# Corleno/Nonstationary_Multivariate_Gaussian_Process

Measured on AMD Instinct MI355X. Metric: log-posterior evals/sec (N=2048, D=3 nonseparable GP), higher is better.
Workload: dtype f64

## Files before the change

nonstationary_multivariate_gaussian_process_amd/csrc/nmgp_chol.hip:

```cpp
#include "nmgp_internal.h"
#include <cstring>

namespace nmgpk {

static inline int cdiv_c(long long a, long long b) { return (int)((a + b - 1) / b); }

typedef double v4d __attribute__((ext_vector_type(4)));

#define SY_BM 128
#define SY_BK 16
#define SY_LD (SY_BM + 16)
#define SY_SB 8

__device__ __forceinline__ int clamp_row_pair(int r, int rows) {
    int rc = r < rows - 1 ? r : rows - 2;
    return rc < 0 ? 0 : rc;
}

__device__ __forceinline__ double fast_recip(double p) {
    double x = __builtin_amdgcn_rcp(p);
    double e = fma(-p, x, 1.0);
    x = fma(x, e, x);
    e = fma(-p, x, 1.0);
    x = fma(x, e, x);
// ... 1542 lines not shown
#pragma unroll
        for (int kk = 0; kk < 4; ++kk) x0 = __builtin_amdgcn_mfma_f64_16x16x4f64(ai[kk], T[pp][kk], x0, 0, 0, 0);
        T[pp] = x0;
#pragma unroll
        for (int kk = 0; kk < 4; ++kk)
#pragma unroll
            for (int q = pp + 1; q < 4; ++q) {
                const double a = reinterpret_cast<const double*>(&ops[(q == 1 ? 0 : (q == 2 ? 1 : 3)) + pp][lane])[kk];
                T[q] = __builtin_amdgcn_mfma_f64_16x16x4f64(a, T[pp][kk], T[q], 0, 0, 0);
            }
    }
    if (v0) {
#pragma unroll
        for (int q = 0; q < 4; ++q)
#pragma unroll
            for (int r = 0; r < 4; ++r) A[(size_t)(16 * q + 4 * r + l4) * lda + row] = T[q][r];
    }
}

static void trsm_64(hipStream_t s, const double* L, int ldl, int nb, double* A, int lda, int rows, int batch,
                    long long bstride, bool precise) {
    if (rows <= 0) return;
    if (precise) {
        NMGP_LAUNCH(k_trsm_64, dim3(cdiv_c(rows, 64), batch), dim3(256), 0, s, L, ldl, nb, A, lda, rows, bstride);
    } else if (nb == 64) {
        NMGP_LAUNCH(k_trsm_64h<5>, dim3(cdiv_c(rows, 64), batch), dim3(256), 0, s, L, ldl, A, lda, rows, bstride);
    } else {
        const long long wgs = (long long)cdiv_c(rows, 128) * batch;
        const int reps = wgs >= 4096 ? 4 : (wgs >= 2048 ? 2 : 1);
        NMGP_LAUNCH(k_trsm_64m, dim3(cdiv_c(rows, 128 * reps), batch), dim3(256), 0, s, L, ldl, nb, A, lda, rows, bstride, reps);
    }
}

#define PS_XLD 66
#define PS_XPS_OFF 6656
#define PS_XS_OFF (PS_XPS_OFF + 64 * PS_XLD)
#define PS_SMEM_DOUBLES (PS_XS_OFF + 64 * PS_XLD)

template <int MODE, int OCC = 2>
__global__ __launch_bounds__(512, OCC) void k_panel_step(double* __restrict__ Ab, int lda, int ck, int has_prev_a,
                                                        int has_next_a,
                                                        int m_act, int pend, long long bstride, int* __restrict__ info,
                                                        int istride, int T, int u_mrows, int u_ncols, int u_kflags,
                                                        int u_tiles, int nbatch, int pre_a, int un_fresh, int u_tri,
                                                        long long* __restrict__ stamps) {
    const int has_prev = MODE == 0 ? has_prev_a : (MODE == 2 ? 1 : 0);
    const int has_next = MODE == 0 ? has_next_a : (MODE == 1 ? 1 : 0);
    const int pre = MODE == 0 ? pre_a : 0;
    constexpr int kOpsT = MODE == 1 ? 0 : 4096;
    constexpr int kXps = PS_XPS_OFF;
    constexpr int kXs = MODE == 1 ? 2560 : PS_XS_OFF;
    constexpr int kSmem = MODE == 1 ? 2560 + 64 * PS_XLD
                                    : (MODE == 2 ? 6656 : (PS_SMEM_DOUBLES > 4 * SY_BK * SY_LD ? PS_SMEM_DOUBLES : 4 * SY_BK * SY_LD));
    static_assert(MODE != 1 || sizeof(Potf2Lds) <= kSmem * sizeof(double), "the factorisation's LDS aliases the step's");
#define PS_STAMP(i)                                                              \
    do {                                                                         \
        if (stamps && blockIdx.x == 0 && threadIdx.x == 0) stamps[i] = (long long)wall_clock64(); \
    } while (0)
    PS_STAMP(0);
    __shared__ __attribute__((aligned(32))) double smem[kSmem];
    const int tid = threadIdx.x, lane = tid & 63, w = tid >> 6;
    const int l15 = lane & 15, l4 = lane >> 4;
    const int bx = (int)blockIdx.x / nbatch, by = (int)blockIdx.x - bx * nbatch;
    if (bx >= T) {
        if constexpr (MODE == 0) {
            const int t = bx - T + by * u_tiles;
            const double* Ap = Ab + (size_t)(ck - 64) * lda + (ck + 128);
            double* Cp = Ab + (size_t)(ck + 128) * lda + (ck + 128);
            syrk_tile_body<4, SY_BK>(Ap, lda, Cp, lda, u_mrows, u_ncols, 64, bstride, bstride, u_kflags, -u_tiles, nbatch, t, 0,
                                     0, smem, smem + 2 * SY_BK * SY_LD, u_tri, 0);
        }
        return;
    }
    double* A = Ab + (size_t)by * bstride;
    v4d* opsC = reinterpret_cast<v4d*>(smem);
    v4d* opsT = reinterpret_cast<v4d*>(smem + kOpsT);
    double* Xps = smem + (MODE == 0 ? kXps : 0);
    double* Xs = smem + (MODE == 2 ? 0 : kXs);
    const bool wg0 = bx == 0;
    const bool isC = wg0 && w < 4;
    const bool wg1 = pre && bx == 1;
    const bool isP = wg1 && w < 4;
    const int row = wg0 ? ck + 64 + 16 * w + l15 : ck + 128 + 128 * (bx - 1) + 16 * w + l15;
    const bool rv = row < m_act && !(wg0 && w >= 4);
    const int rowc = row < m_act ? row : (m_act - 1);
    const bool un_used = has_next && (has_prev || wg0);
    double oc[8], ot[5];
    v4d Xp[4], Tk[4], Un[4];
    const double* Lp = A + (size_t)(ck - 64) * lda;
    if (has_prev) {
#pragma unroll
        for (int j = 0; j < 8; ++j) {
            const int e = tid + 512 * j, q = e >> 10, sx = (e >> 6) & 15, l = e & 63;
            oc[j] = -Lp[(size_t)(4 * sx + (l >> 4)) * lda + ck + 16 * q + (l & 15)];
        }
    }
    {
        const double* L = A + (size_t)ck * lda + ck;
#pragma unroll
        for (int j = 0; j < 5; ++j) {
            const int idx = tid + 512 * j;
            const int blk = idx >> 8, kk = (idx >> 6) & 3, l = idx & 63;
            const int rr = l & 15, kc = 4 * kk + (l >> 4);
            double v;
            if (blk < 6) {
                const int q = blk == 0 ? 1 : (blk < 3 ? 2 : 3);
                const int pp = blk == 0 ? 0 : (blk < 3 ? blk - 1 : blk - 3);
                v = -L[(size_t)(16 * pp + kc) * lda + 16 * q + rr];
            } else {
                const int q = blk - 6;
                if (kc < rr) v = L[(size_t)(16 * q + rr) * lda + 16 * q + kc];
                else if (kc == rr) v = 1.0 / L[(size_t)(16 * q + rr) * lda + 16 * q + rr];
                else v = 0.0;
            }
            ot[j] = v;
        }
    }
    auto load_rows = [&]() {
#pragma unroll
        for (int q = 0; q < 4; ++q)
#pragma unroll
            for (int r = 0; r < 4; ++r) {
                const int c = 16 * q + 4 * r + l4;
                Tk[q][r] = rv ? A[(size_t)(ck + c) * lda + rowc] : 0.0;
                Xp[q][r] = (rv && has_prev) ? Lp[(size_t)c * lda + rowc] : 0.0;
                Un[q][r] = (rv && un_used && row < un_fresh) ? A[(size_t)(ck + 64 + c) * lda + rowc] : 0.0;
            }
    };
    if constexpr (MODE != 2) load_rows();
    if (has_prev) {
#pragma unroll
        for (int j = 0; j < 8; ++j) {
            const int e = tid + 512 * j, q = e >> 10, sx = (e >> 6) & 15, l = e & 63;
            smem[((q * 4 + (sx >> 2)) * 64 + l) * 4 + (sx & 3)] = oc[j];
        }
        if (isP) {
#pragma unroll
            for (int q = 0; q < 4; ++q)
#pragma unroll
                for (int r = 0; r < 4; ++r) Xps[(16 * w + l15) * PS_XLD + 16 * q + 4 * r + l4] = Xp[q][r];
        }
    }
#pragma unroll
    for (int j = 0; j < 5; ++j) {
        const int idx = tid + 512 * j;
        const int blk = idx >> 8, kk = (idx >> 6) & 3, l = idx & 63;
        smem[kOpsT + (blk * 64 + l) * 4 + kk] = ot[j];
    }
    if constexpr (MODE == 2) load_rows();
    __syncthreads();
    PS_STAMP(1);
    if (has_prev && has_next && !wg0) {
#pragma unroll
        for (int j = 0; j < 8; ++j) {
            const int e = tid + 512 * j, q = e >> 10, sx = (e >> 6) & 15, l = e & 63;
            oc[j] = -Lp[(size_t)(4 * sx + (l >> 4)) * lda + ck + 64 + 16 * q + (l & 15)];
        }
    }
    if (has_prev && (!wg0 || isC)) {
#pragma unroll
        for (int sg = 0; sg < 4; ++sg)
#pragma unroll
            for (int kk = 0; kk < 4; ++kk)
#pragma unroll
                for (int q = 0; q < 4; ++q) {
                    const double a = reinterpret_cast<const double*>(&opsC[(q * 4 + sg) * 64 + lane])[kk];
                    Tk[q] = __builtin_amdgcn_mfma_f64_16x16x4f64(a, Xp[sg][kk], Tk[q], 0, 0, 0);
                }
    }
    PS_STAMP(2);
#pragma unroll
    for (int pp = 0; pp < 4; ++pp) {
        const v4d ai = opsT[(6 + pp) * 64 + lane];
        v4d x0 = {0.0, 0.0, 0.0, 0.0};
#pragma unroll
        for (int kk = 0; kk < 4; ++kk) x0 = __builtin_amdgcn_mfma_f64_16x16x4f64(ai[kk], Tk[pp][kk], x0, 0, 0, 0);
        Tk[pp] = x0;
#pragma unroll
        for (int kk = 0; kk < 4; ++kk)
#pragma unroll
            for (int q = pp + 1; q < 4; ++q) {
                const double a = reinterpret_cast<const double*>(&opsT[((q == 1 ? 0 : (q == 2 ? 1 : 3)) + pp) * 64 + lane])[kk];
                Tk[q] = __builtin_amdgcn_mfma_f64_16x16x4f64(a, Tk[pp][kk], Tk[q], 0, 0, 0);
            }
    }
    if (rv) {
#pragma unroll
        for (int q = 0; q < 4; ++q)
#pragma unroll
            for (int r = 0; r < 4; ++r) A[(size_t)(ck + 16 * q + 4 * r + l4) * lda + row] = Tk[q][r];
    }
    PS_STAMP(3);
    if (!has_next) return;
    if (!wg0) {
        if (isP) {
#pragma unroll
            for (int q = 0; q < 4; ++q)
#pragma unroll
                for (int r = 0; r < 4; ++r) Xs[(16 * w + l15) * PS_XLD + 16 * q + 4 * r + l4] = Tk[q][r];
        }
        if (wg1 && !has_prev) __syncthreads();
        if (has_prev) {
            __syncthreads();
#pragma unroll
            for (int j = 0; j < 8; ++j) {
                const int e = tid + 512 * j, q = e >> 10, sx = (e >> 6) & 15, l = e & 63;
                smem[((q * 4 + (sx >> 2)) * 64 + l) * 4 + (sx & 3)] = oc[j];
            }
            __syncthreads();
#pragma unroll
            for (int sg = 0; sg < 4; ++sg)
#pragma unroll
                for (int kk = 0; kk < 4; ++kk)
#pragma unroll
                    for (int q = 0; q < 4; ++q) {
                        const double a = reinterpret_cast<const double*>(&opsC[(q * 4 + sg) * 64 + lane])[kk];
                        Un[q] = __builtin_amdgcn_mfma_f64_16x16x4f64(a, Xp[sg][kk], Un[q], 0, 0, 0);
                    }
        }
        if (rv && (has_prev || row >= un_fresh)) {
#pragma unroll
            for (int q = 0; q < 4; ++q)
#pragma unroll
                for (int r = 0; r < 4; ++r) A[(size_t)(ck + 64 + 16 * q + 4 * r + l4) * lda + row] = Un[q][r];
        }
        if (isP) {
#pragma unroll 1
            for (int q0 = 0; q0 < 4; q0 += 2) {
                v4d Vn[2];
#pragma unroll
                for (int qq = 0; qq < 2; ++qq)
#pragma unroll
                    for (int r = 0; r < 4; ++r) Vn[qq][r] = A[(size_t)(ck + 128 + 16 * (q0 + qq) + 4 * r + l4) * lda + rowc];
                if (has_prev) {
#pragma unroll
                    for (int sg = 0; sg < 4; ++sg)
#pragma unroll
                        for (int kk = 0; kk < 4; ++kk)
#pragma unroll
                            for (int qq = 0; qq < 2; ++qq) {
                                const double a = -Xps[(16 * (q0 + qq) + l15) * PS_XLD + 16 * sg + 4 * kk + l4];
                                const double b = Xps[(16 * w + l15) * PS_XLD + 16 * sg + 4 * kk + l4];
                                Vn[qq] = __builtin_amdgcn_mfma_f64_16x16x4f64(a, b, Vn[qq], 0, 0, 0);
                            }
                }
#pragma unroll
                for (int sg = 0; sg < 4; ++sg)
#pragma unroll
                    for (int kk = 0; kk < 4; ++kk)
#pragma unroll
                        for (int qq = 0; qq < 2; ++qq) {
                            const double a = -Xs[(16 * (q0 + qq) + l15) * PS_XLD + 16 * sg + 4 * kk + l4];
                            const double b = Xs[(16 * w + l15) * PS_XLD + 16 * sg + 4 * kk + l4];
                            Vn[qq] = __builtin_amdgcn_mfma_f64_16x16x4f64(a, b, Vn[qq], 0, 0, 0);
                        }
#pragma unroll
                for (int qq = 0; qq < 2; ++qq)
#pragma unroll
                    for (int r = 0; r < 4; ++r) A[(size_t)(ck + 128 + 16 * (q0 + qq) + 4 * r + l4) * lda + row] = Vn[qq][r];
            }
        }
        return;
    }
    if (isC) {
#pragma unroll
        for (int q = 0; q < 4; ++q)
#pragma unroll
            for (int r = 0; r < 4; ++r) Xs[(16 * w + l15) * PS_XLD + 16 * q + 4 * r + l4] = Tk[q][r];
    }
    PS_STAMP(4);
    __syncthreads();
    PS_STAMP(5);
    if (isC) {
#pragma unroll
        for (int sg = 0; sg < 4; ++sg)
#pragma unroll
            for (int kk = 0; kk < 4; ++kk)
#pragma unroll
                for (int q = 0; q < 4; ++q) {
                    const double a = -Xs[(16 * q + l15) * PS_XLD + 16 * sg + 4 * kk + l4];
                    Un[q] = __builtin_amdgcn_mfma_f64_16x16x4f64(a, Tk[sg][kk], Un[q], 0, 0, 0);
                }
    }
    Potf2Lds& P = *reinterpret_cast<Potf2Lds*>(smem);
    __syncthreads();
    if (isC) {
#pragma unroll
        for (int q = 0; q < 4; ++q)
#pragma unroll
            for (int r = 0; r < 4; ++r) {
                const int rr = 16 * w + l15, cc = 16 * q + 4 * r + l4;
                P.S[cc * PB_LD + rr] = (cc <= rr) ? Un[q][r] : 0.0;
            }
    }
    __syncthreads();
    PS_STAMP(6);
    potf2b_core_mfma(P, info + (size_t)by * istride, ck + 64);
    PS_STAMP(7);
    potf2b_store(A + (size_t)(ck + 64) * lda + (ck + 64), lda, 64, P, tid, 512);
    PS_STAMP(8);
#undef PS_STAMP
}

template <int NP, bool FACT>
__global__ __launch_bounds__(512, 4) void k_leaf_step(double* __restrict__ Ab, int lda, int ck, int m_act, long long bstride,
                                                       int* __restrict__ info, int istride, int T, int nbatch, int t_fresh0,
                                                       int t_fresh1) {
    constexpr int kOpsC = 2560;
    constexpr int kSmem = kOpsC + (FACT ? 64 * PS_XLD : 4096);
    static_assert(64 * PS_XLD >= 4096, "Xs aliases (and covers) the catch-up operands");
    static_assert(!FACT || sizeof(Potf2Lds) <= kSmem * sizeof(double), "the factorisation's LDS aliases the step's");
    static_assert(64 * NP <= 64 * NMGP_XTRI_SEED_BLOCKS, "the catch-up of a row of L^-T would read left of the seeded band");
    __shared__ __attribute__((aligned(32))) double smem[kSmem];
    const int tid = threadIdx.x, lane = tid & 63, w = tid >> 6;
    const int l15 = lane & 15, l4 = lane >> 4;
    const int bx = (int)blockIdx.x / nbatch, by = (int)blockIdx.x - bx * nbatch;
    double* A = Ab + (size_t)by * bstride;
    v4d* opsT = reinterpret_cast<v4d*>(smem);
    v4d* opsC = reinterpret_cast<v4d*>(smem + kOpsC);
    double* Xs = smem + kOpsC;
    const bool wg0 = bx == 0;
    const bool isC = wg0 && w < 4;
    const int row = wg0 ? ck + 64 + 16 * w + l15 : ck + 128 + 128 * (bx - 1) + 16 * w + l15;
    const bool rv = row < m_act && !(wg0 && w >= 4);
    const int rowc = row < m_act ? row : (m_act - 1);
    const bool tload = rv && !(row >= t_fresh0 && row < t_fresh1);
    const int wu = __builtin_amdgcn_readfirstlane(w);
    const unsigned vrow = (unsigned)(l4 * lda + rowc), vops = (unsigned)(l4 * lda + l15);
    auto colp = [&](int col) { return A + (size_t)col * lda; };
    double oc[8], ot[5];
    v4d Xp[4], Tk[4];
    auto load_ops = [&](int p) {
        const int cb = ck - 64 * (NP - p);
#pragma unroll
        for (int j = 0; j < 8; ++j) oc[j] = (colp(cb + 4 * (wu + 8 * (j & 1))) + ck + 16 * (j >> 1))[vops];
    };
    auto store_ops = [&]() {
        __builtin_amdgcn_sched_barrier(0);
#pragma unroll
        for (int j = 0; j < 8; ++j) smem[kOpsC + (((j >> 1) * 4 + (j & 1) * 2 + (wu >> 2)) * 64 + lane) * 4 + (wu & 3)] = -oc[j];
    };
    auto row_block = [&](int cb) { return __builtin_amdgcn_make_buffer_rsrc(colp(cb), (short)0, 0x7fffffff, 0x00020000); };
    auto load_group = [&](v4d& dst, __amdgpu_buffer_rsrc_t blk, int g, unsigned voff) {
#pragma unroll
        for (int r = 0; r < 4; ++r)
            dst[r] = __builtin_bit_cast(double, __builtin_amdgcn_raw_buffer_load_b64(blk, (int)voff, (16 * g + 4 * r) * lda * 8, 0));
    };
    const unsigned kMasked = 0x80000000u;
    const unsigned vxoff = rv ? vrow * 8u : kMasked, vtoff = tload ? vrow * 8u : kMasked;
    load_ops(0);
    {
        const double* L = A + (size_t)ck * lda + ck;
#pragma unroll
        for (int j = 0; j < 5; ++j) {
            const int idx = tid + 512 * j;
            const int blk = idx >> 8, kk = (idx >> 6) & 3, l = idx & 63;
            const int rr = l & 15, kc = 4 * kk + (l >> 4);
            if (j < 3) {
                const int q = blk == 0 ? 1 : (blk < 3 ? 2 : 3);
                const int pp = blk == 0 ? 0 : (blk < 3 ? blk - 1 : blk - 3);
                ot[j] = L[(size_t)(16 * pp + kc) * lda + 16 * q + rr];
            } else {
                const int q = blk - 6;
                ot[j] = L[(size_t)(16 * q + rr) * lda + 16 * q + (kc < rr ? kc : rr)];
            }
        }
    }
    {
        const __amdgpu_buffer_rsrc_t own = row_block(ck), x0 = row_block(ck - 64 * NP);
#pragma unroll
        for (int q = 0; q < 4; ++q) load_group(Tk[q], own, q, vtoff);
#pragma unroll
        for (int q = 0; q < 4; ++q) load_group(Xp[q], x0, q, vxoff);
    }
    store_ops();
#pragma unroll
    for (int j = 0; j < 5; ++j) {
        const int idx = tid + 512 * j;
        const int blk = idx >> 8, kk = (idx >> 6) & 3, l = idx & 63;
        const int rr = l & 15, kc = 4 * kk + (l >> 4);
        const double v = j < 3 ? -ot[j] : (kc < rr ? ot[j] : (kc == rr ? 1.0 / ot[j] : 0.0));
        smem[(blk * 64 + l) * 4 + kk] = v;
    }
    __syncthreads();
#pragma unroll
    for (int p = 0; p < NP; ++p) {
        const bool more = p + 1 < NP;
        if (more) load_ops(p + 1);
        const __amdgpu_buffer_rsrc_t xnext = row_block(ck - 64 * (NP - p - 1));
#pragma unroll
        for (int sg = 0; sg < 4; ++sg) {
            if (!wg0 || isC) {
#pragma unroll
                for (int kk = 0; kk < 4; ++kk)
#pragma unroll
                    for (int q = 0; q < 4; ++q) {
                        const double a = reinterpret_cast<const double*>(&opsC[(q * 4 + sg) * 64 + lane])[kk];
                        Tk[q] = __builtin_amdgcn_mfma_f64_16x16x4f64(a, Xp[sg][kk], Tk[q], 0, 0, 0);
                    }
            }
            if (more) load_group(Xp[sg], xnext, sg, vxoff);
        }
        if (more) {
            __syncthreads();
            store_ops();
            __syncthreads();
        }
    }
#pragma unroll
    for (int pp = 0; pp < 4; ++pp) {
        const v4d ai = opsT[(6 + pp) * 64 + lane];
        v4d x0 = {0.0, 0.0, 0.0, 0.0};
#pragma unroll
        for (int kk = 0; kk < 4; ++kk) x0 = __builtin_amdgcn_mfma_f64_16x16x4f64(ai[kk], Tk[pp][kk], x0, 0, 0, 0);
        Tk[pp] = x0;
#pragma unroll
        for (int kk = 0; kk < 4; ++kk)
#pragma unroll
            for (int q = pp + 1; q < 4; ++q) {
                const double a = reinterpret_cast<const double*>(&opsT[((q == 1 ? 0 : (q == 2 ? 1 : 3)) + pp) * 64 + lane])[kk];
                Tk[q] = __builtin_amdgcn_mfma_f64_16x16x4f64(a, Tk[pp][kk], Tk[q], 0, 0, 0);
            }
    }
    if (rv) {
#pragma unroll
        for (int q = 0; q < 4; ++q)
#pragma unroll
            for (int r = 0; r < 4; ++r) colp(ck + 16 * q + 4 * r)[vrow] = Tk[q][r];
    }
    if constexpr (FACT) {
        if (!wg0) return;
        v4d Un[4];
        if (isC) {
#pragma unroll
            for (int q = 0; q < 4; ++q)
#pragma unroll
                for (int r = 0; r < 4; ++r) Un[q][r] = colp(ck + 64 + 16 * q + 4 * r)[vrow];
        }
#pragma unroll 1
        for (int p = 0; p < NP; ++p) {
            const int cb = ck - 64 * (NP - p);
#pragma unroll
            for (int j = 0; j < 8; ++j) oc[j] = colp(cb + wu + 8 * j)[ck + 64 + lane];
            __syncthreads();
#pragma unroll
            for (int j = 0; j < 8; ++j) Xs[lane * PS_XLD + wu + 8 * j] = oc[j];
            __syncthreads();
            if (isC) {
#pragma unroll
                for (int sg = 0; sg < 4; ++sg)
#pragma unroll
                    for (int kk = 0; kk < 4; ++kk) {
                        const double b = Xs[(16 * w + l15) * PS_XLD + 16 * sg + 4 * kk + l4];
#pragma unroll
                        for (int q = 0; q < 4; ++q) {
                            const double a = -Xs[(16 * q + l15) * PS_XLD + 16 * sg + 4 * kk + l4];
                            Un[q] = __builtin_amdgcn_mfma_f64_16x16x4f64(a, b, Un[q], 0, 0, 0);
                        }
                    }
            }
        }
        __syncthreads();
        if (isC) {
#pragma unroll
            for (int q = 0; q < 4; ++q)
#pragma unroll
                for (int r = 0; r < 4; ++r) Xs[(16 * w + l15) * PS_XLD + 16 * q + 4 * r + l4] = Tk[q][r];
        }
        __syncthreads();
        if (isC) {
#pragma unroll
            for (int sg = 0; sg < 4; ++sg)
#pragma unroll
                for (int kk = 0; kk < 4; ++kk)
#pragma unroll
                    for (int q = 0; q < 4; ++q) {
                        const double a = -Xs[(16 * q + l15) * PS_XLD + 16 * sg + 4 * kk + l4];
                        Un[q] = __builtin_amdgcn_mfma_f64_16x16x4f64(a, Tk[sg][kk], Un[q], 0, 0, 0);
                    }
        }
        Potf2Lds& P = *reinterpret_cast<Potf2Lds*>(smem);
        __syncthreads();
        if (isC) {
#pragma unroll
            for (int q = 0; q < 4; ++q)
#pragma unroll
                for (int r = 0; r < 4; ++r) {
                    const int rr = 16 * w + l15, cc = 16 * q + 4 * r + l4;
                    P.S[cc * PB_LD + rr] = (cc <= rr) ? Un[q][r] : 0.0;
                }
        }
        __syncthreads();
        potf2b_core_mfma(P, info + (size_t)by * istride, ck + 64);
        potf2b_store(A + (size_t)(ck + 64) * lda + (ck + 64), lda, 64, P, tid, 512);
    }
}

__global__ void k_set_row(double* __restrict__ A, int lda, int row, const double* __restrict__ v, int n,
                          long long bstride, long long vstride, int cps) {
    int j = blockIdx.x * blockDim.x + threadIdx.x;
    if (j < n) A[(size_t)blockIdx.y * bstride + (size_t)j * lda + row] = v[(size_t)(blockIdx.y / cps) * vstride + j];
}
void set_row(hipStream_t s, double* A, int lda, int row, const double* v, int n, int batch, long long bstride,
             long long vstride, int cps) {
    NMGP_LAUNCH(k_set_row, dim3(cdiv_c(n, 256), batch), dim3(256), 0, s, A, lda, row, v, n, bstride, vstride, cps < 1 ? 1 : cps);
}
__global__ void k_get_row(const double* __restrict__ A, int lda, int row, double* __restrict__ v, int n,
                          long long bstride, long long vstride) {
    int j = blockIdx.x * blockDim.x + threadIdx.x;
    if (j < n) v[(size_t)blockIdx.y * vstride + j] = A[(size_t)blockIdx.y * bstride + (size_t)j * lda + row];
}
void get_row(hipStream_t s, const double* A, int lda, int row, double* v, int n, int batch, long long bstride,
             long long vstride) {
    NMGP_LAUNCH(k_get_row, dim3(cdiv_c(n, 256), batch), dim3(256), 0, s, A, lda, row, v, n, bstride, vstride);
}

struct Factorisation {
    hipStream_t s, s2;
    double* A;
    int lda, n, extra, xtri;
    int* info;
    int batch;
    long long bs;
    int is;
    bool precise;
    const SyrkHook* hook;
    long long* stamps;
    bool block_done = false;

    double* at(int row, int col) const { return A + (size_t)col * lda + row; }
    int active_rows(int cend) const { return n + extra + (cend < xtri ? cend : xtri); }
    bool take_block_done() {
        const bool done = block_done;
        block_done = false;
        return done;
    }

    void update(hipStream_t st, int c0, int k, int c1, int ncols, int fuse_width) {
        const bool fuse = fuse_width >= 64 && !precise;
        const bool done = syrk_lower(st, at(c1, c0), lda, at(c1, c1), lda, active_rows(c0 + k) - c1, ncols, k, batch, bs, -1, 0,
                                     xtri > 0 ? n + extra - c1 : kNoTriRows, c0, fuse ? info : nullptr, is, c1, hook);
        if (fuse) block_done = done;
    }

    void block_solve(int c0, int w) {
        if (!take_block_done()) potf2_64(s, at(c0, c0), lda, w, info, c0, batch, bs, is, precise);
        trsm_64(s, at(c0, c0), lda, w, at(c0 + w, c0), lda, active_rows(c0 + w) - (c0 + w), batch, bs, precise);
    }

    void fused_steps(int c0, int w, bool leaf) {
        if (!take_block_done()) potf2_64(s, at(c0, c0), lda, 64, info, c0, batch, bs, is, precise);
        const int nk = w / 64;
        for (int k = 0; k < nk; ++k) {
            const int ck = c0 + 64 * k;
            const int m_act = active_rows(ck + 64);
            const int rows = m_act - (ck + 64);
            if (rows <= 0) continue;
            const int has_prev = k > 0, has_next = k + 1 < nk;
            const int T = 1 + (rows > 64 ? cdiv_c(rows - 64, 128) : 0);
            SyrkPlan pl;
            const int u_m = m_act - (ck + 128), u_n = c0 + w - (ck + 128);
            if (has_prev && u_m > 0 && u_n > 0) pl = syrk_plan(lda, lda, u_m, u_n, 64, 1, 0, true);
            const int pre = (ck + 192 <= c0 + w) ? 1 : 0;
            if (pre) pl.kflags |= 128;
            long long* st = stamps ? stamps + (size_t)(ck / 64) * 16 : nullptr;
            const int un_fresh = xtri > 0 ? n + extra + (has_prev ? ck - 64 : ck) : kNoTriRows;
            const int u_tri = xtri > 0 ? n + extra - 64 * NMGP_XTRI_SEED_BLOCKS : kNoTriRows;
            if (leaf && pl.tiles == 0 && !pre && nk == 2) {
                if (k == 0)
                    NMGP_LAUNCH((k_panel_step<1, 4>), dim3((unsigned)(T * batch)), dim3(512), 0, s, A, lda, ck, 0, 1, m_act, c0 + w, bs, info,
                                is, T, 0, 0, 0, 0, batch, 0, un_fresh, u_tri, st);
                else
                    NMGP_LAUNCH((k_panel_step<2, 6>), dim3((unsigned)(T * batch)), dim3(512), 0, s, A, lda, ck, 1, 0, m_act, c0 + w, bs, info,
                                is, T, 0, 0, 0, 0, batch, 0, un_fresh, u_tri, st);
            } else {
                NMGP_LAUNCH((k_panel_step<0, 2>), dim3((unsigned)((T + pl.tiles) * batch)), dim3(512), 0, s, A, lda, ck, has_prev, has_next, m_act,
                            c0 + w, bs, info, is, T, pl.mrows, u_n, pl.kflags, pl.tiles, batch, pre, un_fresh, u_tri, st);
            }
        }
    }

    void leaf256(int c0) {
        if (!take_block_done()) potf2_64(s, at(c0, c0), lda, 64, info, c0, batch, bs, is, precise);
        const int f0 = xtri > 0 ? n + extra + c0 : kNoTriRows;
        for (int k = 0; k < 4; ++k) {
            const int ck = c0 + 64 * k;
            const int m_act = active_rows(ck + 64);
            const int rows = m_act - (ck + 64);
            if (rows <= 0) continue;
            const int T = 1 + (rows > 64 ? cdiv_c(rows - 64, 128) : 0);
            const dim3 grid((unsigned)(T * batch));
            if (k == 0)
                NMGP_LAUNCH((k_panel_step<1, 4>), grid, dim3(512), 0, s, A, lda, ck, 0, 1, m_act, c0 + 128, bs, info, is, T, 0, 0, 0, 0, batch,
                            0, f0, xtri > 0 ? n + extra - 64 * NMGP_XTRI_SEED_BLOCKS : kNoTriRows,
                            stamps ? stamps + (size_t)(ck / 64) * 16 : nullptr);
            else if (k == 1)
                NMGP_LAUNCH((k_leaf_step<1, true>), grid, dim3(512), 0, s, A, lda, ck, m_act, bs, info, is, T, batch, kNoTriRows,
                            kNoTriRows);
            else if (k == 2)
                NMGP_LAUNCH((k_leaf_step<2, true>), grid, dim3(512), 0, s, A, lda, ck, m_act, bs, info, is, T, batch, f0,
                            xtri > 0 ? f0 + 128 : kNoTriRows);
            else
                NMGP_LAUNCH((k_leaf_step<3, false>), grid, dim3(512), 0, s, A, lda, ck, m_act, bs, info, is, T, batch, f0,
                            xtri > 0 ? f0 + 192 : kNoTriRows);
        }
    }

    void panel_rl(int c0, int w) {
        for (int j0 = c0; j0 < c0 + w; j0 += 64) {
            const int jb = (c0 + w - j0 < 64) ? (c0 + w - j0) : 64;
            block_solve(j0, jb);
            update(s, j0, jb, j0 + jb, c0 + w - (j0 + jb), c0 + w - (j0 + jb));
        }
    }

    enum Leaf {
        kBlockSolve,
        kFusedSteps,
        kLeaf128
    };
    void panel_halving(int c0, int w, int base, Leaf leaf) {
        if (w <= base) {
            if (leaf == kBlockSolve || (leaf == kLeaf128 && w != 128)) block_solve(c0, w);
            else fused_steps(c0, w, leaf == kLeaf128);
            return;
        }
        if (leaf == kLeaf128 && w == 256) {
            leaf256(c0);
            return;
        }
        int h = ((w / 2 + 63) / 64) * 64;
        if (h >= w) h = ((w - 1) / 64) * 64;
        panel_halving(c0, h, base, leaf);
        update(s, c0, h, c0 + h, w - h, w - h);
        panel_halving(c0 + h, w - h, base, leaf);
    }

    void panel(int c0, int w) {
        const Switches& sw = switches();
        const bool mfma_ok = w > 0 && (w % 64 == 0) && (lda % 2 == 0) && !precise;
        const bool small = sw.fused_max_batch >= 0 ? batch <= sw.fused_max_batch : (long long)batch * n <= 73728;
        const int rec_min_batch = 4;
        if (mfma_ok && (sw.panel == Switches::kFused || (sw.panel == Switches::kAuto && small)))
            panel_halving(c0, w, fused_base(w), kFusedSteps);
        else if (mfma_ok && sw.panel == Switches::kAuto && batch >= rec_min_batch && w >= 128)
            panel_halving(c0, w, 128, kLeaf128);
        else if (sw.panel == Switches::kRl || (sw.panel != Switches::kRec && batch < rec_min_batch))
            panel_rl(c0, w);
        else
            panel_halving(c0, w, 64, kBlockSolve);
    }
    int fused_base(int w) const {
        if (switches().fused_base >= 64) return switches().fused_base;
        if (w > 256 && (batch >= 16 || (xtri > 0 && batch >= 5))) return 256;
        return w;
    }

    void run(int nb1, hipEvent_t* ev) {
        const bool la = (s2 != nullptr && ev != nullptr && n > 2 * nb1 && batch <= switches().la_max_batch && !precise);
        if (!la) {
            for (int c0 = 0; c0 < n; c0 += nb1) {
                const int w1 = (n - c0 < nb1) ? (n - c0) : nb1;
                const int c1 = c0 + w1;
                panel(c0, w1);
                update(s, c0, w1, c1, n - c1, n - c1 < nb1 ? n - c1 : nb1);
            }
            return;
        }
        hipEventRecord(ev[0], s);
        hipStreamWaitEvent(s2, ev[0], 0);
        int k = 0;
        bool prevB = false;
        for (int c0 = 0; c0 < n; c0 += nb1, ++k) {
            const int w1 = (n - c0 < nb1) ? (n - c0) : nb1;
            const int c1 = c0 + w1;
            const int w1n = (c1 < n) ? ((n - c1 < nb1) ? (n - c1) : nb1) : 0;
            const int c2 = c1 + w1n;
            hipEvent_t evPanel = ev[1 + 2 * k], evB = ev[2 + 2 * k];
            panel(c0, w1);
            if (c1 >= n) break;
            if (prevB) hipStreamWaitEvent(s, ev[2 + 2 * (k - 1)], 0);
            update(s, c0, w1, c1, w1n, w1n);
            hipEventRecord(evPanel, s);
            prevB = false;
            if (c2 < n) {
                hipStreamWaitEvent(s2, evPanel, 0);
                update(s2, c0, w1, c2, n - c2, 0);
                hipEventRecord(evB, s2);
                prevB = true;
            }
        }
        if (prevB) hipStreamWaitEvent(s, ev[2 + 2 * (k - 1)], 0);
    }
};

void potrf_lower(hipStream_t s, hipStream_t s2, hipEvent_t* ev, double* A, int lda, int n, int extra, int xtri,
                 int nb1, int* info, int batch, long long bstride, int istride, const SyrkHook* hook, int precise) {
    if (nb1 <= 0)
        nb1 = (batch >= 16 && n >= 4096) ? 2048
              : (((batch >= 4 && n >= 4096) || (batch >= 32 && n >= 2048)) && (long long)batch * n > 73728) ? 1024 : 512;
    const int nsteps = (n + 63) / 64;
    Factorisation f{s, s2, A, lda, n, extra, xtri, info, batch, bstride, istride, precise != 0, hook, g_step_stamps.begin(s, nsteps)};
    f.run(nb1, ev);
    g_step_stamps.dump(s, nsteps);
}

static_assert(SY_BM + 2 * SY_BK - 2 <= 64 * NMGP_XTRI_SEED_BLOCKS, "update tiles of L^-T rows would read left of the seeded band");
static_assert(NMGP_XTRI_SEED_BLOCKS == 3, "k_panel_step (u_tri) and k_xtri_seed's grid (4 column blocks per row block) assume three seeded blocks");
__global__ __launch_bounds__(256) void k_xtri_seed(double* __restrict__ A, int lda, int row0, int n, int pad,
                                                    long long bstride) {
    A += (size_t)blockIdx.z * bstride;
    const int lane = threadIdx.x & 63, w = threadIdx.x >> 6;
    if (blockIdx.x == gridDim.x - 1) {
        for (int c = blockIdx.y * 256 + threadIdx.x; c < n; c += 256 * gridDim.y)
            for (int q = 0; q < pad; ++q) A[(size_t)c * lda + row0 + q] = 0.0;
        return;
    }
    const int b = blockIdx.x;
    const int r = 64 * b + lane;
    const int cb = b - NMGP_XTRI_SEED_BLOCKS + (int)blockIdx.y;
    if (cb < 0 || r >= n) return;
#pragma unroll 4
    for (int k = 0; k < 16; ++k) {
        const int c = 64 * cb + w + 4 * k;
        if (c < n) A[(size_t)c * lda + row0 + pad + r] = (r == c) ? 1.0 : 0.0;
    }
}
void identity_rows(hipStream_t s, double* A, int lda, int row0, int n, int pad, int batch, long long bstride) {
    NMGP_LAUNCH(k_xtri_seed, dim3(cdiv_c(n, 64) + 1, NMGP_XTRI_SEED_BLOCKS + 1, batch), dim3(256), 0, s, A, lda, row0, n, pad, bstride);
}

}
```

Baseline: 1775.

## Fuse leaf-256 Cholesky steps into fewer kernels with a paired trailing update

```diff
diff --git a/nonstationary_multivariate_gaussian_process_amd/csrc/nmgp_chol.hip b/nonstationary_multivariate_gaussian_process_amd/csrc/nmgp_chol.hip
--- a/nonstationary_multivariate_gaussian_process_amd/csrc/nmgp_chol.hip
+++ b/nonstationary_multivariate_gaussian_process_amd/csrc/nmgp_chol.hip
@@ -1868,29 +1868,20 @@
 #undef PS_STAMP
 }
 
-template <int NP, bool FACT>
-__global__ __launch_bounds__(512, 4) void k_leaf_step(double* __restrict__ Ab, int lda, int ck, int m_act, long long bstride,
-                                                       int* __restrict__ info, int istride, int T, int nbatch, int t_fresh0,
-                                                       int t_fresh1) {
-    constexpr int kOpsC = 2560;
-    constexpr int kSmem = kOpsC + (FACT ? 64 * PS_XLD : 4096);
+#define LS_OPSC 2560
+#define LS_SMEM (LS_OPSC + 64 * PS_XLD)
+template <int NP>
+__device__ __forceinline__ void leaf_step_body(double* A, int lda, int ck, int* info, double* smem,
+                                               int tid, int rowc, bool rv, bool act, bool isC, bool crit) {
+    constexpr int kOpsC = LS_OPSC;
     static_assert(64 * PS_XLD >= 4096, "Xs aliases (and covers) the catch-up operands");
-    static_assert(!FACT || sizeof(Potf2Lds) <= kSmem * sizeof(double), "the factorisation's LDS aliases the step's");
-    static_assert(64 * NP <= 64 * NMGP_XTRI_SEED_BLOCKS, "the catch-up of a row of L^-T would read left of the seeded band");
-    __shared__ __attribute__((aligned(32))) double smem[kSmem];
-    const int tid = threadIdx.x, lane = tid & 63, w = tid >> 6;
+    static_assert(sizeof(Potf2Lds) <= LS_SMEM * sizeof(double), "the factorisation's LDS aliases the step's");
+    const int lane = tid & 63, w = tid >> 6;
     const int l15 = lane & 15, l4 = lane >> 4;
-    const int bx = (int)blockIdx.x / nbatch, by = (int)blockIdx.x - bx * nbatch;
-    double* A = Ab + (size_t)by * bstride;
     v4d* opsT = reinterpret_cast<v4d*>(smem);
     v4d* opsC = reinterpret_cast<v4d*>(smem + kOpsC);
     double* Xs = smem + kOpsC;
-    const bool wg0 = bx == 0;
-    const bool isC = wg0 && w < 4;
-    const int row = wg0 ? ck + 64 + 16 * w + l15 : ck + 128 + 128 * (bx - 1) + 16 * w + l15;
-    const bool rv = row < m_act && !(wg0 && w >= 4);
-    const int rowc = row < m_act ? row : (m_act - 1);
-    const bool tload = rv && !(row >= t_fresh0 && row < t_fresh1);
+    const bool tload = rv;
     const int wu = __builtin_amdgcn_readfirstlane(w);
     const unsigned vrow = (unsigned)(l4 * lda + rowc), vops = (unsigned)(l4 * lda + l15);
     auto colp = [&](int col) { return A + (size_t)col * lda; };
@@ -1916,7 +1907,7 @@
     const unsigned vxoff = rv ? vrow * 8u : kMasked, vtoff = tload ? vrow * 8u : kMasked;
     load_ops(0);
     {
-        const double* L = A + (size_t)ck * lda + ck;
+        const double* L = colp(ck) + ck;
 #pragma unroll
         for (int j = 0; j < 5; ++j) {
             const int idx = tid + 512 * j;
@@ -1925,10 +1916,10 @@
             if (j < 3) {
                 const int q = blk == 0 ? 1 : (blk < 3 ? 2 : 3);
                 const int pp = blk == 0 ? 0 : (blk < 3 ? blk - 1 : blk - 3);
-                ot[j] = L[(size_t)(16 * pp + kc) * lda + 16 * q + rr];
+                ot[j] = L[(unsigned)((16 * pp + kc) * lda + 16 * q + rr)];
             } else {
                 const int q = blk - 6;
-                ot[j] = L[(size_t)(16 * q + rr) * lda + 16 * q + (kc < rr ? kc : rr)];
+                ot[j] = L[(unsigned)((16 * q + rr) * lda + 16 * q + (kc < rr ? kc : rr))];
             }
         }
     }
@@ -1956,7 +1947,7 @@
         const __amdgpu_buffer_rsrc_t xnext = row_block(ck - 64 * (NP - p - 1));
 #pragma unroll
         for (int sg = 0; sg < 4; ++sg) {
-            if (!wg0 || isC) {
+            if (act) {
 #pragma unroll
                 for (int kk = 0; kk < 4; ++kk)
 #pragma unroll
@@ -1994,8 +1985,8 @@
 #pragma unroll
             for (int r = 0; r < 4; ++r) colp(ck + 16 * q + 4 * r)[vrow] = Tk[q][r];
     }
-    if constexpr (FACT) {
-        if (!wg0) return;
+    {
+        if (!crit) return;
         v4d Un[4];
         if (isC) {
 #pragma unroll
@@ -2057,8 +2048,197 @@
                 }
         }
         __syncthreads();
-        potf2b_core_mfma(P, info + (size_t)by * istride, ck + 64);
+        potf2b_core_mfma(P, info, ck + 64);
         potf2b_store(A + (size_t)(ck + 64) * lda + (ck + 64), lda, 64, P, tid, 512);
+    }
+}
+
+__global__ __launch_bounds__(512, 4) void k_leaf_step(double* Ab, int lda, int ck, int m_act, long long bstride, int* info,
+                                                       int istride, int nbatch) {
+    __shared__ __attribute__((aligned(32))) double smem[LS_SMEM];
+    const int tid = threadIdx.x, lane = tid & 63, w = tid >> 6;
+    const int l15 = lane & 15;
+    const int bx = (int)blockIdx.x / nbatch, by = (int)blockIdx.x - bx * nbatch;
+    double* A = Ab + (size_t)by * bstride;
+    int* infob = info + (size_t)by * istride;
+    const bool wg0 = bx == 0;
+    const int wu = __builtin_amdgcn_readfirstlane(w);
+    const int row = wg0 ? ck + 64 + 16 * w + l15 : ck + 192 + 128 * (bx - 1) + 16 * w + l15;
+    const bool rv = row < m_act;
+    const int rowc = rv ? row : (m_act - 1);
+    leaf_step_body<1>(A, lda, ck, infob, smem, tid, rowc, rv, true, wg0 && wu < 4, wg0);
+    if (!wg0) return;
+    __syncthreads();
+    int t2 = tid;
+    asm volatile("" : "+v"(t2));
+    const bool c2 = __builtin_amdgcn_readfirstlane(t2 >> 6) < 4;
+    leaf_step_body<2>(A, lda, ck + 64, infob, smem, t2, ck + 128 + 16 * ((t2 >> 6) & 3) + (t2 & 15), c2, c2, c2, true);
+}
+
+__global__ __launch_bounds__(512, 4) void k_leaf_pair(double* __restrict__ Ab, int lda, int c2, int m_act2, int m_act3,
+                                                       long long bstride, int nbatch, int f0) {
+    constexpr int kT2 = 4096, kT3 = kT2 + 2560, kSmem = kT3 + 2560;
+    static_assert(kSmem * sizeof(double) <= 80 * 1024, "two workgroups per CU");
+    static_assert(64 * 3 <= 64 * NMGP_XTRI_SEED_BLOCKS, "the catch-up of a row of L^-T would read left of the seeded band");
+    __shared__ __attribute__((aligned(32))) double smem[kSmem];
+    const int tid = threadIdx.x, lane = tid & 63, w = tid >> 6;
+    const int l15 = lane & 15, l4 = lane >> 4;
+    const int bx = (int)blockIdx.x / nbatch, by = (int)blockIdx.x - bx * nbatch;
+    double* A = Ab + (size_t)by * bstride;
+    const int row = c2 + 128 + 128 * bx + 16 * w + l15;
+    const bool rv3 = row < m_act3, rv2 = row < m_act2;
+    const int rowc = rv3 ? row : (m_act3 - 1);
+    const bool tl2 = rv2 && !((unsigned)(row - f0) < 128u), tl3 = rv3 && !((unsigned)(row - f0) < 192u);
+    const int wu = __builtin_amdgcn_readfirstlane(w);
+    const unsigned vrow = (unsigned)(l4 * lda + rowc), vops = (unsigned)(l4 * lda + l15);
+    auto colp = [&](int col) { return A + (size_t)col * lda; };
+    auto row_block = [&](int cb) { return __builtin_amdgcn_make_buffer_rsrc(colp(cb), (short)0, 0x7fffffff, 0x00020000); };
+    auto load_group = [&](v4d& dst, __amdgpu_buffer_rsrc_t blk, int g, unsigned voff) {
+#pragma unroll
+        for (int r = 0; r < 4; ++r)
+            dst[r] = __builtin_bit_cast(double, __builtin_amdgcn_raw_buffer_load_b64(blk, (int)voff, (16 * g + 4 * r) * lda * 8, 0));
+    };
+    const unsigned kMasked = 0x80000000u;
+    const unsigned vxoff = rv3 ? vrow * 8u : kMasked, vt2off = tl2 ? vrow * 8u : kMasked, vt3off = tl3 ? vrow * 8u : kMasked;
+    constexpr int kNX = 3;
+    constexpr bool kAhead = false;
+    double og[4], ot[5];
+    v4d Xp[kNX], Tk2[4], Tk3[4];
+    auto load_gops = [&](int i) {
+#pragma unroll
+        for (int q = 0; q < 4; ++q) og[q] = (colp(c2 - 128 + 16 * i + 4 * (wu & 3)) + c2 + 64 * (wu >> 2) + 16 * q)[vops];
+    };
+    auto store_gops = [&](int buf) {
+        __builtin_amdgcn_sched_barrier(0);
+#pragma unroll
+        for (int q = 0; q < 4; ++q) smem[2048 * buf + (((wu >> 2) * 4 + q) * 64 + lane) * 4 + (wu & 3)] = -og[q];
+    };
+    auto load_ot = [&](int cd, int t) {
+        const double* L = colp(cd) + cd;
+#pragma unroll
+        for (int j = 0; j < 5; ++j) {
+            const int idx = t + 512 * j;
+            const int blk = idx >> 8, kk = (idx >> 6) & 3, l = idx & 63;
+            const int rr = l & 15, kc = 4 * kk + (l >> 4);
+            if (j < 3) {
+                const int q = blk == 0 ? 1 : (blk < 3 ? 2 : 3);
+                const int pp = blk == 0 ? 0 : (blk < 3 ? blk - 1 : blk - 3);
+                ot[j] = L[(unsigned)((16 * pp + kc) * lda + 16 * q + rr)];
+            } else {
+                const int q = blk - 6;
+                ot[j] = L[(unsigned)((16 * q + rr) * lda + 16 * q + (kc < rr ? kc : rr))];
+            }
+        }
+    };
+    auto store_ot = [&](int base, int t) {
+#pragma unroll
+        for (int j = 0; j < 5; ++j) {
+            const int idx = t + 512 * j;
+            const int blk = idx >> 8, kk = (idx >> 6) & 3, l = idx & 63;
+            const int rr = l & 15, kc = 4 * kk + (l >> 4);
+            const double v = j < 3 ? -ot[j] : (kc < rr ? ot[j] : (kc == rr ? 1.0 / ot[j] : 0.0));
+            smem[base + (blk * 64 + l) * 4 + kk] = v;
+        }
+    };
+    auto solve = [&](v4d (&T)[4], const v4d* opsT) {
+#pragma unroll
+        for (int pp = 0; pp < 4; ++pp) {
+            const v4d ai = opsT[(6 + pp) * 64 + lane];
+            v4d x0 = {0.0, 0.0, 0.0, 0.0};
+#pragma unroll
+            for (int kk = 0; kk < 4; ++kk) x0 = __builtin_amdgcn_mfma_f64_16x16x4f64(ai[kk], T[pp][kk], x0, 0, 0, 0);
+            T[pp] = x0;
+#pragma unroll
+            for (int kk = 0; kk < 4; ++kk)
+#pragma unroll
+                for (int q = pp + 1; q < 4; ++q) {
+                    const double a = reinterpret_cast<const double*>(&opsT[((q == 1 ? 0 : (q == 2 ? 1 : 3)) + pp) * 64 + lane])[kk];
+                    T[q] = __builtin_amdgcn_mfma_f64_16x16x4f64(a, T[pp][kk], T[q], 0, 0, 0);
+                }
+        }
+    };
+    load_gops(0);
+    load_ot(c2, tid);
+    {
+        const __amdgpu_buffer_rsrc_t own2 = row_block(c2), own3 = row_block(c2 + 64), x0 = row_block(c2 - 128);
+#pragma unroll
+        for (int q = 0; q < 4; ++q) load_group(Tk2[q], own2, q, vt2off);
+#pragma unroll
+        for (int q = 0; q < 4; ++q) load_group(Tk3[q], own3, q, vt3off);
+#pragma unroll
+        for (int g = 0; g < kNX; ++g) load_group(Xp[g], x0, g, vxoff);
+    }
+    store_gops(0);
+    store_ot(kT2, tid);
+    __syncthreads();
+    double o32[8];
+    int t7 = tid;
+#pragma unroll
+    for (int i = 0; i < 8; ++i) {
+        if (i < 7) {
+            load_gops(i + 1);
+        } else {
+#pragma unroll
+            for (int j = 0; j < 8; ++j) o32[j] = (colp(c2 + 4 * (wu + 8 * (j & 1))) + c2 + 64 + 16 * (j >> 1))[vops];
+            asm volatile("" : "+v"(t7));
+            load_ot(c2 + 64, t7);
+        }
+        const v4d* g = reinterpret_cast<const v4d*>(smem + 2048 * (i & 1)) + lane;
+        v4d a = g[0];
+#pragma unroll
+        for (int tq = 0; tq < 8; ++tq) {
+            v4d an = a;
+            if (tq < 7) an = g[(tq + 1) * 64];
+            if (kAhead) __builtin_amdgcn_sched_barrier(0);
+            v4d& acc = tq < 4 ? Tk2[tq & 3] : Tk3[tq & 3];
+#pragma unroll
+            for (int kk = 0; kk < 4; ++kk) acc = __builtin_amdgcn_mfma_f64_16x16x4f64(a[kk], Xp[i % kNX][kk], acc, 0, 0, 0);
+            __builtin_amdgcn_sched_barrier(0);
+            a = an;
+        }
+        if (i + kNX < 8) load_group(Xp[i % kNX], row_block(c2 - 128 + 64 * ((i + kNX) >> 2)), (i + kNX) & 3, vxoff);
+        if (i < 7) {
+            store_gops((i + 1) & 1);
+            __syncthreads();
+        }
+    }
+    __syncthreads();
+    __builtin_amdgcn_sched_barrier(0);
+#pragma unroll
+    for (int j = 0; j < 8; ++j) smem[(((j >> 1) * 4 + (j & 1) * 2 + (wu >> 2)) * 64 + lane) * 4 + (wu & 3)] = -o32[j];
+    store_ot(kT3, t7);
+    solve(Tk2, reinterpret_cast<const v4d*>(smem + kT2));
+#pragma unroll
+    for (int q = 0; q < 4; ++q)
+#pragma unroll
+        for (int r = 0; r < 4; ++r) Tk2[q][r] = rv2 ? Tk2[q][r] : 0.0;
+    if (rv2) {
+#pragma unroll
+        for (int q = 0; q < 4; ++q)
+#pragma unroll
+            for (int r = 0; r < 4; ++r) colp(c2 + 16 * q + 4 * r)[vrow] = Tk2[q][r];
+    }
+    __syncthreads();
+    {
+        const v4d* opsC = reinterpret_cast<const v4d*>(smem) + lane;
+        v4d a = opsC[0];
+#pragma unroll
+        for (int e = 0; e < 16; ++e) {
+            v4d an = a;
+            if (e < 15) an = opsC[(((e + 1) & 3) * 4 + ((e + 1) >> 2)) * 64];
+            if (kAhead) __builtin_amdgcn_sched_barrier(0);
+#pragma unroll
+            for (int kk = 0; kk < 4; ++kk) Tk3[e & 3] = __builtin_amdgcn_mfma_f64_16x16x4f64(a[kk], Tk2[e >> 2][kk], Tk3[e & 3], 0, 0, 0);
+            __builtin_amdgcn_sched_barrier(0);
+            a = an;
+        }
+    }
+    solve(Tk3, reinterpret_cast<const v4d*>(smem + kT3));
+    if (rv3) {
+#pragma unroll
+        for (int q = 0; q < 4; ++q)
+#pragma unroll
+            for (int r = 0; r < 4; ++r) colp(c2 + 64 + 16 * q + 4 * r)[vrow] = Tk3[q][r];
     }
 }
 
@@ -2149,26 +2329,25 @@
     void leaf256(int c0) {
         if (!take_block_done()) potf2_64(s, at(c0, c0), lda, 64, info, c0, batch, bs, is, precise);
         const int f0 = xtri > 0 ? n + extra + c0 : kNoTriRows;
-        for (int k = 0; k < 4; ++k) {
-            const int ck = c0 + 64 * k;
-            const int m_act = active_rows(ck + 64);
-            const int rows = m_act - (ck + 64);
-            if (rows <= 0) continue;
-            const int T = 1 + (rows > 64 ? cdiv_c(rows - 64, 128) : 0);
-            const dim3 grid((unsigned)(T * batch));
-            if (k == 0)
-                NMGP_LAUNCH((k_panel_step<1, 4>), grid, dim3(512), 0, s, A, lda, ck, 0, 1, m_act, c0 + 128, bs, info, is, T, 0, 0, 0, 0, batch,
-                            0, f0, xtri > 0 ? n + extra - 64 * NMGP_XTRI_SEED_BLOCKS : kNoTriRows,
-                            stamps ? stamps + (size_t)(ck / 64) * 16 : nullptr);
-            else if (k == 1)
-                NMGP_LAUNCH((k_leaf_step<1, true>), grid, dim3(512), 0, s, A, lda, ck, m_act, bs, info, is, T, batch, kNoTriRows,
-                            kNoTriRows);
-            else if (k == 2)
-                NMGP_LAUNCH((k_leaf_step<2, true>), grid, dim3(512), 0, s, A, lda, ck, m_act, bs, info, is, T, batch, f0,
-                            xtri > 0 ? f0 + 128 : kNoTriRows);
-            else
-                NMGP_LAUNCH((k_leaf_step<3, false>), grid, dim3(512), 0, s, A, lda, ck, m_act, bs, info, is, T, batch, f0,
-                            xtri > 0 ? f0 + 192 : kNoTriRows);
+        {
+            const int m_act = active_rows(c0 + 64);
+            const int T = 1 + cdiv_c(m_act - (c0 + 128), 128);
+            NMGP_LAUNCH((k_panel_step<1, 4>), dim3((unsigned)(T * batch)), dim3(512), 0, s, A, lda, c0, 0, 1, m_act, c0 + 128, bs, info, is,
+                        T, 0, 0, 0, 0, batch, 0, f0, xtri > 0 ? n + extra - 64 * NMGP_XTRI_SEED_BLOCKS : kNoTriRows,
+                        stamps ? stamps + (size_t)(c0 / 64) * 16 : nullptr);
+        }
+        {
+            const int m_act = active_rows(c0 + 128);
+            const int below = m_act - (c0 + 256);
+            const int T = 1 + (below > 0 ? cdiv_c(below, 128) : 0);
+            NMGP_LAUNCH(k_leaf_step, dim3((unsigned)(T * batch)), dim3(512), 0, s, A, lda, c0 + 64, m_act, bs, info, is, batch);
+        }
+        {
+            const int m_act2 = active_rows(c0 + 192), m_act3 = active_rows(c0 + 256);
+            const int below = m_act3 - (c0 + 256);
+            if (below > 0)
+                NMGP_LAUNCH(k_leaf_pair, dim3((unsigned)(cdiv_c(below, 128) * batch)), dim3(512), 0, s, A, lda, c0 + 128, m_act2, m_act3,
+                            bs, batch, f0);
         }
     }
 
```

After: 1789, median of 6. Within noise of the previous version (+0.8%).
